# rimelq/VISTAF-RoboSkin-Vision-Integrated-Multimodal-Sensor

Hardware: AMD Instinct MI355X
Metric: frames/sec (224x224 -> force-map) at batch 256 (higher is better)
Workload: dtype f32; 1 GPU; BASELINE configs[2]: batch 256/GPU of 224x224x3 fp16 fringe frames (256 distinct frames) -> 224x224 f32 depth map + force scalars, full FTP path (inpaint, demod, unwrap, detrend, compose, force tail), constants scaled-224; inputs resident in HBM; global_batch=256, input_dtype=fp16, constants=scaled, parallelism=dp1, inflight_batches=3, frames_with_nonzero_status=0

## Files before the change

vistaf-roboskin-vision-integrated-multimodal-sensor_amd/_lib.py:

```python
from __future__ import annotations

import ctypes
import os

_HERE = os.path.dirname(os.path.abspath(__file__))
LIB_PATH = os.path.join(_HERE, "libvistaf_ftp.so")

NSCALARS = 16
NREFINFO = 8
NCONTACT = 16
MAX_CONTACTS = 64
NTRACK = 16
TRACK_NAMES = ["track_id", "age_frames", "parent_row", "events", "overlap_px", "dx", "dy", "dforce_N", "dvolume_cm3", "origin_track_id"]
TRACK_EVENTS = {"born": 1, "split": 2, "merged": 4, "gated": 8}
FATE_ENDED, FATE_NO_ROW = -1, -2 ** 31
NSHAPE = 24
SHAPE_NAMES = ["contact_pixels", "boundary_pixels", "footprint_cx", "footprint_cy", "major_axis_mm", "minor_axis_mm", "orientation_rad",
               "fit_pixels", "fit_status", "apex_x", "apex_y", "apex_depth_mm", "curvature_1_per_mm", "curvature_2_per_mm",
               "curvature_axis_rad", "radius_1_mm", "radius_2_mm", "fit_rms_mm"]
SHAPE_FIT = {"ok": 0, "none": 1, "not_a_cap": 2}
NTAXEL, NTAXELFRAME, TAXEL_NONE = 12, 8, 0xFFFF
TAXEL_NAMES = ["contact_pixels", "contact_area_mm2", "volume_cm3", "mean_depth_mm", "max_depth_mm", "argmax_index", "centroid_x", "centroid_y",
               "force_N", "pressure_kPa"]
TAXEL_FRAME_NAMES = ["active_taxels", "volume_cm3", "force_N", "cop_x", "cop_y", "moment_x_Nmm", "moment_y_Nmm", "peak_taxel"]
NTHERMAL, NTHERMALFRAME = 16, 8
THERMAL_NAMES = ["contact_pixels", "valid_pixels", "coverage", "mean_C", "weighted_mean_C", "min_C", "max_C", "std_C", "peak_temp_C",
                 "surround_pixels", "surround_mean_C", "contrast_C"]
THERMAL_FRAME_NAMES = ["registered_pixels", "skin_mean_C", "contact_pixels", "contact_mean_C", "contrast_C", "hottest_contact", "coldest_contact"]
ALIGN_NINFO = 12

FMT_GRAY_U8, FMT_BGR_U8, FMT_GRAY_F16, FMT_BGR_F16 = 0, 1, 2, 3
FRAME_OK, FRAME_EMPTY_RELIABLE, FRAME_QUEUE_OVERFLOW, FRAME_NO_CARRIER = 0, 1, 2, 3
CURVE_TYPES = {"linear0": 0, "linear": 1, "poly2": 2, "sat_exp": 3, "growth": 4, "hinge_saturating": 5}

EXPORTS = [
    "vistaf_ftp_abi_version", "vistaf_ftp_last_error", "vistaf_ftp_default_config", "vistaf_ftp_create",
    "vistaf_ftp_set_reference", "vistaf_ftp_get_reference_info", "vistaf_ftp_predict_batch", "vistaf_ftp_predict_pairs",
    "vistaf_ftp_get_pair_info", "vistaf_ftp_contacts",
    "vistaf_ftp_get_intermediate", "vistaf_ftp_stage_count", "vistaf_ftp_stage_name",
    "vistaf_ftp_enable_stage_timing", "vistaf_ftp_get_stage_times", "vistaf_ftp_destroy",
    "vistaf_depth_map_to_volume", "vistaf_predict_force_from_volume",
]
TEST_EXPORTS = ["vistaf_ftp_test_set", "vistaf_ftp_test_select", "vistaf_ftp_test_polyfit", "vistaf_ftp_test_gauss",
                "vistaf_ftp_test_chamfer"]
TEMP_EXPORTS = ["vistaf_tempseg_default_config", "vistaf_tempseg_create", "vistaf_tempseg_destroy", "vistaf_tempseg_segment",
                "vistaf_temp_feature_planes", "vistaf_temp_color_support",
                "vistaf_temp_clamp_map", "vistaf_temp_inpaint_map", "vistaf_temp_fuse_maps", "vistaf_temp_oriented_blur"]
TEMPSEG_NINFO = 16
TEMPMODEL_EXPORTS = ["vistaf_tmodel_create", "vistaf_tmodel_destroy", "vistaf_tmodel_predict_maps", "vistaf_tmodel_predict_rows"]
TSENSOR_EXPORTS = ["vistaf_tsensor_default_config", "vistaf_tsensor_create", "vistaf_tsensor_destroy", "vistaf_tsensor_predict",
                   "vistaf_tsensor_stats_create", "vistaf_tsensor_stats_destroy", "vistaf_tsensor_map_statistics"]
TSENSOR_NINFO, TSENSOR_NMASKS, TSENSOR_NSTATS = TEMPSEG_NINFO + 4, 5, 6
TRACK_EXPORTS = ["vistaf_track_create", "vistaf_track_update", "vistaf_track_reset", "vistaf_track_destroy"]
SHAPE_EXPORTS = ["vistaf_shape_create", "vistaf_shape_measure", "vistaf_shape_destroy"]
TAXEL_EXPORTS = ["vistaf_taxel_create", "vistaf_taxel_measure", "vistaf_taxel_layout_info", "vistaf_taxel_destroy"]
THERMAL_EXPORTS = ["vistaf_thermal_create", "vistaf_thermal_register", "vistaf_thermal_measure", "vistaf_thermal_destroy"]
ALIGN_EXPORTS = [
    "vistaf_align_default_config", "vistaf_align_create", "vistaf_align_destroy", "vistaf_align_geometry",
    "vistaf_align_set_reference", "vistaf_align_batch",
]


class Curve(ctypes.Structure):
    _fields_ = [("type", ctypes.c_int32), ("reserved", ctypes.c_int32),
                ("a", ctypes.c_double), ("b", ctypes.c_double), ("c", ctypes.c_double)]

# ... 49 lines not shown
    lib.vistaf_ftp_abi_version.restype = ci
    lib.vistaf_ftp_last_error.restype = ctypes.c_char_p
    lib.vistaf_ftp_default_config.argtypes = [ctypes.POINTER(CConfig)]
    lib.vistaf_ftp_create.argtypes = [ctypes.POINTER(CConfig), ci, ci, ci, ci, ci, ci, ctypes.POINTER(Curve), ci,
                                      ctypes.POINTER(Curve), ctypes.POINTER(vp)]
    lib.vistaf_ftp_set_reference.argtypes = [vp, vp, ci, vp]
    lib.vistaf_ftp_get_reference_info.argtypes = [vp, ctypes.POINTER(cd)]
    lib.vistaf_ftp_predict_batch.argtypes = [vp, vp, ci, ci, vp, vp, vp, vp, vp]
    lib.vistaf_ftp_predict_pairs.argtypes = [vp, vp, vp, ci, ci, vp, vp, vp, vp, vp]
    lib.vistaf_ftp_get_pair_info.argtypes = [vp, ci, ctypes.POINTER(cd), vp]
    lib.vistaf_ftp_contacts.argtypes = [vp, ci, ci, vp, vp, vp, vp]
    lib.vistaf_ftp_get_intermediate.argtypes = [vp, ctypes.c_char_p, vp, ci, ctypes.POINTER(ctypes.c_size_t), vp]
    lib.vistaf_ftp_stage_count.restype = ci
    lib.vistaf_ftp_stage_name.restype = ctypes.c_char_p
    lib.vistaf_ftp_stage_name.argtypes = [ci]
    lib.vistaf_ftp_enable_stage_timing.argtypes = [vp, ci]
    lib.vistaf_ftp_get_stage_times.argtypes = [vp, ctypes.POINTER(ctypes.c_float), ci]
    lib.vistaf_ftp_destroy.argtypes = [vp]
    lib.vistaf_ftp_destroy.restype = None
    lib.vistaf_depth_map_to_volume.argtypes = [vp, vp, ci, ci, ci, cd, cd, vp, vp]
    lib.vistaf_predict_force_from_volume.argtypes = [ctypes.POINTER(Curve), cd, ctypes.POINTER(cd)]
    lib.vistaf_ftp_test_set.argtypes = [vp, ctypes.c_char_p, ci]
    lib.vistaf_ftp_test_select.argtypes = [vp, vp, ctypes.c_size_t, vp, ci, vp, ci, vp, vp, ci, ci, ci, vp]
    lib.vistaf_ftp_test_polyfit.argtypes = [vp, vp, ci, ci, ctypes.c_float, ci, ci, vp, vp, ci, ci, ci, ci, vp]
    lib.vistaf_ftp_test_gauss.argtypes = [vp, vp, cd, ci, ci, ci, vp]
    lib.vistaf_ftp_test_chamfer.argtypes = [vp, ci, ci, vp, vp, ci, ci, ci, ci, vp]
    lib.vistaf_tempseg_default_config.argtypes = [ctypes.POINTER(CTempSegConfig)]
    lib.vistaf_tempseg_create.argtypes = [ctypes.POINTER(CTempSegConfig), ci, ci, ctypes.POINTER(vp)]
    lib.vistaf_tempseg_destroy.argtypes = [vp]
    lib.vistaf_tempseg_destroy.restype = None
    lib.vistaf_tempseg_segment.argtypes = [vp, vp, vp, vp, vp, vp, vp, ctypes.POINTER(cd), vp]
    lib.vistaf_temp_feature_planes.argtypes = [vp, vp, ci, vp, vp, vp, vp, vp]
    lib.vistaf_temp_color_support.argtypes = [vp, vp, vp, vp, vp, vp, cd, ci, vp, vp, vp]
    lib.vistaf_temp_clamp_map.argtypes = [vp, vp, vp, cd, cd, vp, vp]
    lib.vistaf_temp_inpaint_map.argtypes = [vp, vp, vp, ci, vp, vp]
    lib.vistaf_temp_fuse_maps.argtypes = [vp, vp, vp, vp, ctypes.POINTER(CTempFuseConfig), vp, vp, ctypes.POINTER(ctypes.c_int64), vp]
    lib.vistaf_temp_oriented_blur.argtypes = [vp, vp, vp, cd, cd, cd, vp, vp]
    i32p, dp = ctypes.POINTER(ctypes.c_int32), ctypes.POINTER(cd)
    lib.vistaf_tmodel_create.argtypes = [ci, i32p, dp, dp, ci, ci, ci, i32p, dp, cd, ci, dp, dp, cd, cd, ci, ctypes.POINTER(vp)]
    lib.vistaf_tmodel_destroy.argtypes = [vp]
    lib.vistaf_tmodel_destroy.restype = None
    lib.vistaf_tmodel_predict_maps.argtypes = [ci, ctypes.POINTER(vp), ctypes.POINTER(vp), ctypes.POINTER(vp), ctypes.POINTER(vp), ctypes.c_int64,
                                               ctypes.c_int64, vp]
    lib.vistaf_tmodel_predict_rows.argtypes = [vp, vp, ci, ctypes.c_int64, vp, vp]
    lib.vistaf_tsensor_default_config.argtypes = [ctypes.POINTER(CTSensorConfig)]
    lib.vistaf_tsensor_create.argtypes = [ctypes.POINTER(CTSensorConfig), ci, ci, vp, vp, ctypes.POINTER(vp)]
# ... 40 lines not shown
```

vistaf-roboskin-vision-integrated-multimodal-sensor_amd/csrc/api.hip:

```cpp
#include <hip/hip_runtime.h>
#include <algorithm>
#include <cmath>
#include <cstdio>
#include <cstdlib>
#include <cstring>
#include <map>
#include <string>
#include <vector>

#include "host_util.hpp"

using namespace vf;
#include "test_hooks.h"
#ifdef VISTAF_DEBUG
namespace vf { void telea_debug_dump(); void telea_window_debug_dump(int B); void telea_window_mw_debug_dump(int B); void fit_debug_dump(); void unwrap_big_debug_dump(); void unwrap_batch_debug_dump(); }
#endif

static thread_local std::string g_err;
static int fail(int code, const std::string &msg) { g_err = msg; return code; }
namespace vf { int set_error(int code, const std::string &msg) { return fail(code, msg); } }

namespace {

struct GKern { float *d = nullptr; int k = 0; };
// ... 35 lines not shown
    struct Named { void *p; size_t bytes; bool per_frame; };
    std::map<std::string, Named> named;
    DeviceAllocs allocs;
    float *img, *grad, *tmpf, *blurA, *inorm, *iw, *amp, *prod, *quality, *wrapped, *unwrapped, *phase1, *resid0, *detr, *z0, *mplane,
        *num, *den, *hmap, *dist, *z0f, *snum, *unitless, *depth;
    double2 *field, *patch;
    double2 *tmpT;
    uint8_t *bad0, *bad1, *rel0, *rel1, *rel2, *reliable, *contact, *contact_d, *background, *cand, *kept;
    uint8_t *out_rel = nullptr, *hole_cand = nullptr;
    float *hole_med = nullptr, *hole_fill = nullptr;
    int32_t *labels, *area, *rowdist, *parent;
    unsigned int *peak_bits;
    uint16_t *morph_pre;
    void *inpaint_scratch, *inpaint_cl_scratch, *inpaint_win_scratch, *unwrap_scratch;
    void *big_scratch = nullptr;
    int32_t *unwrap_need;
    float *thr_hi, *thr_g, *mu, *amp_thr, *thr3, *thr_used, *bg_med, *core_thr, *core_med, *coef;
    int *cnt_a, *cnt_valid, *rel_count, *contact_count, *bg_count, *bad_count, *flipped;
    unsigned int *gmax;
    int32_t *status;
    int32_t *big_only;
    unsigned long long *cc_best;
    double *scalars;
    float *req_hi, *req_g, *req_med, *req_amp, *req_contact, *req_core;

    ContactScratch contacts_ws{};
    int last_batch = 0;
    bool last_pairs = false;

    bool timing = false;
    hipEvent_t ev[ST_COUNT + 1];
    bool ev_made = false;
    float stage_ms[ST_COUNT];
};

namespace {

template <typename T>
int dalloc(vistaf_ftp_handle *hd, T **p, size_t count, const char *name = nullptr, size_t per_frame = 0)
{
    const int rc = hd->allocs.alloc(p, count);
    if (!rc && name) hd->named[name] = {*p, per_frame, true};
    return rc;
}

int make_gkern(vistaf_ftp_handle *hd, double sigma, GKern *g)
{
// ... 49 lines not shown
void *chain_scratch(const vistaf_ftp_handle *hd) { return hd->tiers.big_chain ? hd->big_scratch : nullptr; }

float q32_of(double pct) { return (float)pct / 100.0f; }

int upload_req(vistaf_ftp_handle *hd, float **d, const std::vector<float> &v)
{
    int rc = dalloc(hd, d, v.size());
    if (rc) return rc;
    if (hipMemcpy(*d, v.data(), v.size() * sizeof(float), hipMemcpyHostToDevice) != hipSuccess) return fail(VISTAF_E_HIP, "memcpy req");
    return 0;
}

void preprocess(vistaf_ftp_handle *hd, const void *frames, int format, int nframes, hipStream_t st, bool timed, const void *frames2 = nullptr)
{
    const vistaf_ftp_config &c = hd->cfg;
    int h = hd->h, w = hd->w, P = hd->P;
    if (timed) hipEventRecord(hd->ev[ST_GRAY_BAD], st);
    launch_to_gray(frames, format, hd->img, nframes, P, st);
    if (frames2) launch_to_gray(frames2, format, hd->img + (size_t)nframes * P, nframes, P, st);
    const int B = frames2 ? 2 * nframes : nframes;
    hipMemsetAsync(hd->bad_count, 0, sizeof(int) * B, st);
    if (c.bad_pixel_enable) {
        launch_sobel_mag(hd->img, hd->grad, B, h, w, st);
        launch_select(hd->img, hd->valid, 0, nullptr, false, hd->req_hi, 1, hd->thr_hi, hd->cnt_valid, B, P, st, chain_scratch(hd));
        launch_select(hd->grad, hd->valid, 0, nullptr, false, hd->req_g, 1, hd->thr_g, nullptr, B, P, st, chain_scratch(hd));
        launch_bad_flags(hd->img, hd->grad, hd->valid, hd->thr_hi, hd->thr_g, hd->bad0, B, P, st);
        uint8_t *src = hd->bad0, *dst = hd->bad1;
        if (c.bad_dilate_ksize > 1)
            for (int it = 0; it < c.bad_dilate_iters; it++) { launch_morph(src, dst, B, h, w, hd->se_bad, true, nullptr, nullptr, st); std::swap(src, dst); }
        if (src != hd->bad1) hipMemcpyAsync(hd->bad1, src, (size_t)B * P, hipMemcpyDeviceToDevice, st);
        launch_count_u8(hd->bad1, hd->bad_count, B, P, st);
        {
            int range = std::min(100, std::max(1, cv_round((double)c.bad_inpaint_radius)));
            const uint8_t *seq_mask = hd->bad1;
            const int32_t *only = nullptr;
            int mode = hd->tiers.inpaint;
            if (mode == 2 && (size_t)h * w > (size_t)8 * 14464) mode = 0;
            if (mode == 0 && inpaint_clusters_supported(range)) {
                uint8_t *bad_big = nullptr;
                ClusterPlanes left;
                launch_inpaint_clusters(hd->img, hd->bad1, range, hd->inpaint_cl_scratch, &bad_big, &left, B, h, w, st);
                if (timed) hipEventRecord(hd->ev[ST_INPAINT], st);
                launch_inpaint_big_clusters(hd->img, bad_big, range, hd->inpaint_scratch, hd->status, left, B, h, w, st, hd->tiers.big_queue_lds != 0,
                                            hd->tiers.big_gq_cap);
                if (hd->tiers.big_fallback) {
                    launch_inpaint_big_handback(hd->status, hd->big_only, B, st);
                    launch_inpaint_telea(hd->img, bad_big, range, hd->inpaint_scratch, hd->status, hd->big_only, B, h, w, st);
                }
            } else {
                if (timed && mode == 1) hipEventRecord(hd->ev[ST_INPAINT], st);
                if (mode != 1) only = launch_inpaint_window(hd->img, seq_mask, range, hd->inpaint_win_scratch, B, h, w, st, timed ? hd->ev[ST_INPAINT] : nullptr,
                                                               hd->tiers.telea_two_tier != 0, hd->tiers.telea_mw != 0);
                launch_inpaint_telea(hd->img, seq_mask, range, hd->inpaint_scratch, hd->status, only, B, h, w, st);
            }
        }
    } else if (timed) hipEventRecord(hd->ev[ST_INPAINT], st);
    if (timed) hipEventRecord(hd->ev[ST_PREPROC], st);
    blur(hd, hd->img, hd->blurA, hd->g_illum, B, st);
    if (fuses(hd, hd->g_pre)) launch_illum_pre_apod(hd->img, hd->blurA, hd->apo, hd->iw, hd->g_pre.d, hd->g_pre.k, B, h, w, st);
    else {
        launch_illum_norm(hd->img, hd->blurA, hd->inorm, B, P, st);
        const float *in = hd->inorm;
        if (hd->g_pre.k) { blur(hd, hd->inorm, hd->blurA, hd->g_pre, B, st); in = hd->blurA; }
        launch_mul_static(in, hd->apo, hd->iw, B, P, st);
    }
    launch_select(hd->iw, hd->valid, 0, nullptr, false, hd->req_med, 1, hd->mu, nullptr, B, P, st, chain_scratch(hd));
}

std::vector<float> hann_patch(int ph, int pw)
{
    auto hann = [](int M, int i) -> float { return M == 1 ? 1.0f : (float)(0.5 + 0.5 * std::cos(3.14159265358979323846 * (double)(1 - M + 2 * i) / (double)(M - 1))); };
    std::vector<float> win((size_t)ph * pw);
    for (int a = 0; a < ph; a++)
        for (int c = 0; c < pw; c++) win[(size_t)a * pw + c] = hann(ph, a) * hann(pw, c);
    return win;
}

PostParams post_params(const vistaf_ftp_handle *hd, const CarrierGeom *pair_geom)
{
    PostParams pp;
    pp.mm_per_px = hd->mm_per_px; pp.depth_eps_mm = hd->cfg.depth_eps_mm; pp.period_px = hd->period; pp.force_curve = hd->fcurve;
    pp.pair_geom = pair_geom; pp.grating_pitch_mm = hd->cfg.grating_pitch_mm;
    return pp;
}

void ensure_events(vistaf_ftp_handle *hd)
{
    if (hd->ev_made) return;
    for (int i = 0; i <= ST_COUNT; i++) hipEventCreate(&hd->ev[i]);
// ... 142 lines not shown
    TRY(dalloc(hd, &hd->thr3, mb * 3)); TRY(dalloc(hd, &hd->thr_used, mb)); TRY(dalloc(hd, &hd->bg_med, mb));
    TRY(dalloc(hd, &hd->core_thr, mb)); TRY(dalloc(hd, &hd->core_med, mb)); TRY(dalloc(hd, &hd->coef, mb * 6));
    TRY(dalloc(hd, &hd->cnt_a, mb)); TRY(dalloc(hd, &hd->cnt_valid, mb)); TRY(dalloc(hd, &hd->rel_count, mb));
    TRY(dalloc(hd, &hd->contact_count, mb)); TRY(dalloc(hd, &hd->bg_count, mb)); TRY(dalloc(hd, &hd->bad_count, mb));
    TRY(dalloc(hd, &hd->flipped, mb)); TRY(dalloc(hd, &hd->gmax, mb)); TRY(dalloc(hd, &hd->status, mb)); TRY(dalloc(hd, &hd->cc_best, mb));
    TRY(dalloc(hd, &hd->big_only, mb));
    TRY(dalloc(hd, &hd->scalars, mb * VISTAF_NSCALARS));
    TRY(dalloc(hd, &hd->hole_med, mb)); TRY(dalloc(hd, &hd->hole_fill, mb));
    {
        ContactScratch &cs = hd->contacts_ws;
        cs.cap = contact_root_capacity(h, w);
        TRY(dalloc(hd, &cs.arg, n)); TRY(dalloc(hd, &cs.list, mb * cs.cap)); TRY(dalloc(hd, &cs.nroots, mb)); TRY(dalloc(hd, &cs.nsel, mb));
        TRY(dalloc(hd, &cs.selkey, mb * VISTAF_MAX_CONTACTS)); TRY(dalloc(hd, &cs.part, contact_part_words(max_batch, P)));
    }
    hd->named["mu"] = {hd->mu, sizeof(float), true}; hd->named["thr_hi"] = {hd->thr_hi, sizeof(float), true}; hd->named["thr_g"] = {hd->thr_g, sizeof(float), true};
    hd->named["coef"] = {hd->coef, 6 * sizeof(float), true}; hd->named["thr3"] = {hd->thr3, 3 * sizeof(float), true};
    hd->named["core_thr"] = {hd->core_thr, sizeof(float), true}; hd->named["core_med"] = {hd->core_med, sizeof(float), true};
    TRY(upload_req(hd, &hd->req_hi, {q32_of(cfg->bad_intensity_percentile)}));
    TRY(upload_req(hd, &hd->req_g, {q32_of(cfg->bad_gradient_percentile)}));
    TRY(upload_req(hd, &hd->req_med, {-1.0f}));
    TRY(upload_req(hd, &hd->req_amp, {q32_of(cfg->amp_valid_percentile)}));
    TRY(upload_req(hd, &hd->req_contact, {q32_of(cfg->contact_percentile), q32_of(95.0), q32_of(98.0)}));
    TRY(upload_req(hd, &hd->req_core, {q32_of(cfg->contact_core_percentile)}));
    TRY(dalloc(hd, &hd->roi_den, (size_t)P));
    if (hd->g_unrel.k) {
        float *tmp_roi = nullptr;
        TRY(upload(hd, &tmp_roi, roif));
        launch_gauss_rows(tmp_roi, hd->tmpf, hd->g_unrel.d, hd->g_unrel.k, 1, h, w, 0);
        launch_gauss_cols(hd->tmpf, hd->roi_den, hd->g_unrel.d, hd->g_unrel.k, 1, h, w, 0);
        std::vector<float> hden(P);
        if (hipMemcpy(hden.data(), hd->roi_den, P * sizeof(float), hipMemcpyDeviceToHost) != hipSuccess) { vistaf_ftp_destroy(hd); return fail(VISTAF_E_HIP, "roi_den readback"); }
        for (int i = 0; i < P; i++) hden[i] = hden[i] + 1e-6f;
        if (hipMemcpy(hd->roi_den, hden.data(), P * sizeof(float), hipMemcpyHostToDevice) != hipSuccess) { vistaf_ftp_destroy(hd); return fail(VISTAF_E_HIP, "roi_den upload"); }
    }
    hd->Hf = h + 2 * std::max(0, cfg->fft_pad_px);
    hd->Wf = w + 2 * std::max(0, cfg->fft_pad_px);
    if (hipDeviceSynchronize() != hipSuccess) { vistaf_ftp_destroy(hd); return fail(VISTAF_E_HIP, "create sync"); }
#undef TRY
    *out = hd;
    return 0;
}

static int reference_search(vistaf_ftp_handle *hd, int nb, CarrierGeom *geom_dev, hipStream_t st)
{
    const vistaf_ftp_config &c = hd->cfg;
    const int h = hd->h, w = hd->w, Hf = hd->Hf, Wf = hd->Wf, pad = std::max(0, c.fft_pad_px);
// ... 55 lines not shown
    return 0;
}

int vistaf_ftp_get_reference_info(const vistaf_ftp_handle *hd, double *o)
{
    if (!hd || !o) return fail(VISTAF_E_INVALID, "null argument");
    if (!hd->have_ref) return fail(VISTAF_E_STATE, "set_reference has not been called");
    o[0] = hd->peak_x; o[1] = hd->peak_y; o[2] = hd->kx; o[3] = hd->ky; o[4] = hd->Hf; o[5] = hd->Wf; o[6] = hd->period; o[7] = hd->mm_per_px;
    return 0;
}

static int post_demod(vistaf_ftp_handle *hd, int B, float *d_height_mm, uint8_t *d_reliable, double *d_scalars, int32_t *d_status,
                      const CarrierGeom *pair_geom, hipStream_t st, const int *bad_count = nullptr)
{
    if (!bad_count) bad_count = hd->bad_count;
    const vistaf_ftp_config &c = hd->cfg;
    int h = hd->h, w = hd->w, P = hd->P;
    bool timed = hd->timing;

    if (timed) hipEventRecord(hd->ev[ST_RELIABLE], st);
    if (hd->g_qual.k) blur(hd, hd->prod, hd->quality, hd->g_qual, B, st);
    else HIPCHK(hipMemcpyAsync(hd->quality, hd->prod, (size_t)B * P * sizeof(float), hipMemcpyDeviceToDevice, st));
    const float *qual = hd->quality;
    launch_select(qual, hd->roi, 0, nullptr, false, hd->req_amp, 1, hd->amp_thr, nullptr, B, P, st, chain_scratch(hd));
    launch_threshold_mask(qual, hd->roi, hd->amp_thr, hd->rel0, B, P, st);
    {
        uint8_t *src = hd->rel0, *dst = hd->rel1;
        if (c.valid_close_iters >= 1 && 2 * c.valid_close_iters <= 4) {
            int ops[4];
            for (int it = 0; it < c.valid_close_iters; it++) { ops[it] = 1; ops[c.valid_close_iters + it] = 0; }
            launch_morph_seq(hd->rel0, hd->rel1, hd->rel2, B, h, w, hd->se_close, ops, 2 * c.valid_close_iters, hd->roi, nullptr, st, hd->morph_pre);
            src = hd->rel1;
        } else {
            for (int it = 0; it < 2 * c.valid_close_iters; it++) {
                const bool dil = it < c.valid_close_iters;
                launch_morph(src, dst, B, h, w, hd->se_close, dil, it == 2 * c.valid_close_iters - 1 ? hd->roi : nullptr, nullptr, st, hd->morph_pre);
                src = dst;
                dst = dst == hd->rel1 ? hd->rel2 : hd->rel1;
            }
        }
        launch_cc_label(src, hd->labels, B, h, w, st);
        launch_cc_largest(hd->labels, hd->area, hd->cc_best, hd->roi, hd->rel2, B, P, st);
    }
    if (c.reliable_edge_margin_px > 0) {
        RowSpanSE ball;
        if (chamfer_ball((float)c.reliable_edge_margin_px, &ball))
            launch_morph(hd->rel2, hd->reliable, B, h, w, ball, false, nullptr, nullptr, st, hd->morph_pre);
        else {
            launch_chamfer(hd->rel2, false, hd->rowdist, hd->dist, B, h, w, c.reliable_edge_margin_px + 1, st, hd->tiers.chamfer_twopass != 0);
            launch_erode_by_dist(hd->dist, hd->rel2, (float)c.reliable_edge_margin_px, hd->reliable, B, P, st);
        }
    } else HIPCHK(hipMemcpyAsync(hd->reliable, hd->rel2, (size_t)B * P, hipMemcpyDeviceToDevice, st));
    launch_count_u8(hd->reliable, hd->rel_count, B, P, st);
    launch_mark_empty(hd->rel_count, hd->status, B, st);

    if (timed) hipEventRecord(hd->ev[ST_UNWRAP_RANK], st);
    launch_unwrap(hd->wrapped, qual, hd->reliable, hd->unwrapped, hd->parent, hd->unwrap_scratch, hd->status, B, h, w, st,
                  timed ? hd->ev[ST_UNWRAP_TREE] : nullptr, timed ? hd->ev[ST_UNWRAP] : nullptr, hd->tiers.big_flood_handback != 0, hd->tiers.unwrap_fast ? hd->unwrap_need : nullptr);

    if (timed) hipEventRecord(hd->ev[ST_DETREND], st);
    if (c.plane_order_for_removal > 0)
        launch_robust_polyfit(hd->unwrapped, hd->reliable, c.plane_order_for_removal, c.irls_iters, (float)c.irls_c, 200, 500, hd->coef, hd->phase1, B, h, w, st, chain_scratch(hd));
    else
        HIPCHK(hipMemcpyAsync(hd->phase1, hd->unwrapped, (size_t)B * P * sizeof(float), hipMemcpyDeviceToDevice, st));
    launch_robust_polyfit(hd->phase1, hd->reliable, c.poly_order, c.irls_iters, (float)c.irls_c, 200, 0, hd->coef, hd->resid0, B, h, w, st, chain_scratch(hd));
    launch_select(hd->resid0, hd->reliable, (size_t)P, nullptr, true, hd->req_contact, 3, hd->thr3, nullptr, B, P, st, chain_scratch(hd));
    launch_contact_mask(hd->resid0, hd->reliable, hd->thr3, hd->rel_count, hd->contact_count, c.min_contact_frac, c.max_contact_frac,
                        hd->contact, hd->thr_used, B, P, st);
    {
        int iters = c.dilate_iters;
        if (iters <= 0) HIPCHK(hipMemcpyAsync(hd->contact_d, hd->contact, (size_t)B * P, hipMemcpyDeviceToDevice, st));
        else if (iters <= 4) {
            int ops[4] = {1, 1, 1, 1};
            launch_morph_seq(hd->contact, hd->contact_d, hd->cand, B, h, w, hd->se_contact, ops, iters, nullptr, hd->reliable, st, hd->morph_pre);
        } else {
            uint8_t *src = hd->contact, *dst = hd->contact_d;
            uint8_t *bufs[2] = {hd->contact_d, hd->cand};
            for (int it = 0; it < iters; it++) {
                dst = bufs[it & 1];
                launch_morph(src, dst, B, h, w, hd->se_contact, true, nullptr, it == iters - 1 ? hd->reliable : nullptr, st, hd->morph_pre);
                src = dst;
            }
            if (src != hd->contact_d) HIPCHK(hipMemcpyAsync(hd->contact_d, src, (size_t)B * P, hipMemcpyDeviceToDevice, st));
        }
    }
    launch_background(hd->reliable, hd->contact_d, hd->rel_count, hd->bg_count, hd->background, B, P, st);
    launch_robust_polyfit(hd->phase1, hd->background, c.poly_order, c.irls_iters, (float)c.irls_c, 200, 0, hd->coef, hd->detr, B, h, w, st, chain_scratch(hd));
    launch_select(hd->detr, hd->background, (size_t)P, nullptr, false, hd->req_med, 1, hd->bg_med, nullptr, B, P, st, chain_scratch(hd));

    if (timed) hipEventRecord(hd->ev[ST_SMOOTH_FLIP], st);
    const bool smooth_rel = hd->g_rel.k > 0;
    if (fuses(hd, hd->g_rel)) launch_smooth_reliable(hd->detr, hd->bg_med, hd->reliable, hd->hmap, hd->g_rel.d, hd->g_rel.k, B, h, w, st);
    else if (smooth_rel) {
        launch_sub_scalar_mask(hd->detr, hd->bg_med, hd->reliable, hd->z0, hd->mplane, B, P, st);
        blur(hd, hd->z0, hd->num, hd->g_rel, B, st);
        blur(hd, hd->mplane, hd->den, hd->g_rel, B, st);
        launch_div_planes(hd->num, hd->den, hd->hmap, B, P, st);
    } else launch_zeroed_keep_nan(hd->detr, hd->bg_med, hd->reliable, hd->hmap, B, P, st);
    launch_select(hd->hmap, hd->reliable, (size_t)P, nullptr, false, hd->req_core, 1, hd->core_thr, nullptr, B, P, st, chain_scratch(hd));
    launch_select(hd->hmap, hd->reliable, (size_t)P, hd->core_thr, false, hd->req_med, 1, hd->core_med, nullptr, B, P, st, chain_scratch(hd));
    launch_core_flip(hd->hmap, hd->core_med, hd->flipped, B, P, st);

    const uint8_t *orel = hd->reliable;
    if (!smooth_rel) {
        const int ksz = std::max(3, c.hole_neighborhood_px | 1);
        launch_chamfer(hd->reliable, false, hd->rowdist, hd->dist, B, h, w, c.hole_min_dist_px + 1, st, hd->tiers.chamfer_twopass != 0);
        launch_hole_candidates(hd->hmap, hd->reliable, hd->dist, ksz, (float)c.hole_known_fraction, (float)c.hole_min_dist_px, hd->hole_cand, B, h, w, st);
        launch_select(hd->hmap, hd->reliable, (size_t)P, nullptr, false, hd->req_med, 1, hd->hole_med, nullptr, B, P, st, chain_scratch(hd));
        launch_hole_tmp(hd->hmap, hd->reliable, hd->hole_cand, hd->hole_med, hd->z0, B, P, st);
        launch_select(hd->z0, hd->reliable, (size_t)P, nullptr, false, hd->req_med, 1, hd->hole_fill, nullptr, B, P, st, chain_scratch(hd));
        launch_hole_zin(hd->z0, hd->hole_fill, B, P, st);
        {
            const int range = std::min(100, std::max(1, cv_round((double)c.inpaint_radius)));
            const int32_t *only = nullptr;
            if (hd->tiers.inpaint != 1) only = launch_inpaint_window(hd->z0, hd->hole_cand, range, hd->inpaint_win_scratch, B, h, w, st, nullptr, hd->tiers.telea_two_tier != 0, hd->tiers.telea_mw != 0);
            launch_inpaint_telea(hd->z0, hd->hole_cand, range, hd->inpaint_scratch, hd->status, only, B, h, w, st);
        }
        launch_hole_merge(hd->hmap, hd->reliable, hd->hole_cand, hd->z0, hd->out_rel, B, P, st);
        orel = hd->out_rel;
    }

    if (timed) hipEventRecord(hd->ev[ST_COMPOSE], st);
    bool use_band = c.frontier_zero_band_px > 0;
    float band = (float)c.frontier_zero_band_px;
    if (use_band) launch_chamfer_pair(orel, hd->rowdist, hd->dist, hd->area, hd->depth, B, h, w, c.frontier_zero_band_px + 2, st, hd->tiers.chamfer_twopass != 0);
    else HIPCHK(hipMemsetAsync(hd->dist, 0x7f, (size_t)B * P * sizeof(float), st));
    const bool fuse_compose = fuses(hd, hd->g_unrel);
    if (fuse_compose)
        launch_compose_finalize_mm(hd->hmap, orel, hd->roi, hd->dist, use_band ? band : 1.0f, hd->roi_den, use_band ? hd->depth : hd->dist, band,
                                   use_band ? 1 : 0, hd->hcurve, hd->use_neg, hd->unitless, hd->depth, hd->cand, hd->gmax, hd->g_unrel.d, hd->g_unrel.k,
                                   B, h, w, st);
    else {
        launch_frontier_compose(hd->hmap, orel, hd->roi, hd->dist, use_band ? band : 1.0f, hd->z0f, B, P, st);
// ... 158 lines not shown
    return 0;
}
int vistaf_ftp_get_stage_times(vistaf_ftp_handle *hd, float *ms_out, int n)
{
    if (!hd || !ms_out) return fail(VISTAF_E_INVALID, "null argument");
    for (int i = 0; i < n && i < ST_COUNT; i++) ms_out[i] = hd->stage_ms[i];
    return 0;
}

int vistaf_ftp_test_set(vistaf_ftp_handle *hd, const char *name, int value)
{
    if (!hd || !name) return fail(VISTAF_E_INVALID, "null argument");
    const std::string n(name);
    if (n == "inpaint_tier" && value >= 0 && value <= 2) hd->tiers.inpaint = value;
    else if (n == "big_flood_handback") hd->tiers.big_flood_handback = value != 0;
    else if (n == "chamfer_twopass") hd->tiers.chamfer_twopass = value != 0;
    else if (n == "telea_two_tier") hd->tiers.telea_two_tier = value != 0;
    else if (n == "telea_mw") hd->tiers.telea_mw = value != 0;
    else if (n == "big_queue_lds") hd->tiers.big_queue_lds = value != 0;
    else if (n == "big_gq_cap" && (value == 0 || (value >= 64 && (value & (value - 1)) == 0))) hd->tiers.big_gq_cap = value;
    else if (n == "big_fallback") hd->tiers.big_fallback = value != 0;
    else if (n == "unwrap_fast") hd->tiers.unwrap_fast = value != 0;
    else if (n == "big_chain") hd->tiers.big_chain = value != 0;
    else if (n == "fused_chains") hd->tiers.fused_chains = value != 0;
    else if (n == "fused_backend") hd->tiers.fused_backend = value != 0;
    else if (n == "keep_planes") hd->keep_planes = value != 0;
    else return fail(VISTAF_E_INVALID, "unknown test hook or value: " + n);
    return 0;
}

namespace {
int hook_scratch(int variant, int B, int h, int w, bool chain_ok, void **scratch)
{
    *scratch = nullptr;
    if (variant < 0 || variant > 2) return fail(VISTAF_E_INVALID, "variant must be 0, 1 or 2");
    if (variant == 2 && !chain_ok) return fail(VISTAF_E_INVALID, "variant 2: the k_big.hip chain does not take this batch");
    if (variant == 1 || (variant == 0 && (size_t)h * w < 262144)) return 0;
    HIPCHK(hipMalloc(scratch, big_scratch_bytes(B, h, w) + 256));
    return 0;
}
int hook_finish(void *a, void *b, hipStream_t st)
{
    const hipError_t e1 = hipGetLastError(), e2 = hipStreamSynchronize(st);
    if (a) (void)hipFree(a);
    if (b) (void)hipFree(b);
    if (e1 != hipSuccess) return fail(VISTAF_E_HIP, std::string("launch: ") + hipGetErrorString(e1));
    if (e2 != hipSuccess) return fail(VISTAF_E_HIP, std::string("sync: ") + hipGetErrorString(e2));
    return 0;
}
}

int vistaf_ftp_test_select(const float *vals, const uint8_t *mask, size_t mask_stride, const float *le_thr, int use_abs, const float *reqs, int nreq,
                           float *out, int *counts, int B, int P, int variant, void *stream)
{
    if (!vals || !mask || !reqs || !out || B < 1 || P < 1 || nreq < 1 || (mask_stride != 0 && mask_stride != (size_t)P))
        return fail(VISTAF_E_INVALID, "bad argument");
    void *scratch = nullptr;
    int rc = hook_scratch(variant, B, 1, P, nreq <= 4 && big_frames(B, P), &scratch);
    if (rc) return rc;
    launch_select(vals, mask, mask_stride, le_thr, use_abs != 0, reqs, nreq, out, counts, B, P, (hipStream_t)stream, scratch);
    return hook_finish(scratch, nullptr, (hipStream_t)stream);
}

int vistaf_ftp_test_polyfit(const float *z, const uint8_t *mask, int order, int iters, float c, int min_count, int min_mask_count, float *coef,
                            float *resid, int B, int h, int w, int variant, void *stream)
{
    if (!z || !mask || !coef || !resid || B < 1 || h < 1 || w < 1 || (size_t)h * w > 0x7fffffffull || order < 1 || order > 2 || iters < 1)
        return fail(VISTAF_E_INVALID, "bad argument");
    void *scratch = nullptr;
    int rc = hook_scratch(variant, B, h, w, big_frames(B, h * w), &scratch);
    if (rc) return rc;
    const int inst = polyfit_variant(B, h, w, scratch != nullptr);
    launch_robust_polyfit(z, mask, order, iters, c, min_count, min_mask_count, coef, resid, B, h, w, (hipStream_t)stream, scratch);
    rc = hook_finish(scratch, nullptr, (hipStream_t)stream);
    return rc ? rc : inst;
}

int vistaf_ftp_test_gauss(const float *src, float *dst, double sigma, int B, int h, int w, void *stream)
{
    if (!src || !dst || src == dst || B < 1 || h < 1 || w < 1 || !(sigma > 0)) return fail(VISTAF_E_INVALID, "bad argument");
    if (gauss_ksize(sigma) > 511) return fail(VISTAF_E_INVALID, "gaussian sigma too large (ksize > 511)");
    const std::vector<float> f = gauss_taps(sigma);
    float *taps = nullptr, *tmp = nullptr;
    HIPCHK(hipMalloc((void **)&taps, f.size() * sizeof(float)));
// ... 44 lines not shown
```

vistaf-roboskin-vision-integrated-multimodal-sensor_amd/csrc/k_select.hip:

```cpp
#include "kernels.hpp"
#include "select.hpp"

namespace vf {

struct PlaneGetter {
    const float *v; const uint8_t *m; float le; bool use_le, use_abs;
    __device__ bool operator()(int i, uint32_t &key) const
    {
        const uint8_t mk = m[i];
        float x = v[i];
        bool ok = mk != 0 && finitef(x);
        if (use_abs) x = fabsf(x);
        if (use_le && !(x <= le)) ok = false;
        key = f2key(x);
        return ok;
    }
};

__global__ __launch_bounds__(SEL_T) void k_select(const float *__restrict__ vals, const uint8_t *__restrict__ mask, size_t mask_stride,
                                                  const float *__restrict__ le_thr, int use_abs, const float *__restrict__ reqs,
                                                  int nreq, float *__restrict__ out, int *__restrict__ counts, int P)
{
    __shared__ SelShared sh;
    size_t b = blockIdx.x;
    PlaneGetter g{vals + b * (size_t)P, mask + b * mask_stride, le_thr ? le_thr[b] : 0.f, le_thr != nullptr, use_abs != 0};
    uint32_t n, kmin, kmax;
    block_minmax(g, P, sh, n, kmin, kmax);
    if (threadIdx.x == 0 && counts) counts[b] = (int)n;
    for (int j = 0; j < nreq; j++) {
        float q = reqs[j];
        float r = (q < 0.f) ? block_median(g, P, sh, n, kmin, kmax) : block_percentile(g, P, q, sh, n, kmin, kmax);
        if (threadIdx.x == 0) out[b * (size_t)nreq + j] = r;
        __syncthreads();
    }
}

void launch_select(const float *vals, const uint8_t *mask, size_t mask_stride, const float *le_thr, bool use_abs,
                   const float *reqs_dev, int nreq, float *out, int *counts, int B, int P, hipStream_t st, void *big_scratch)
{
    if (big_scratch && nreq <= 4 && big_frames(B, P)) {
        launch_select_big(vals, mask, mask_stride, le_thr, use_abs, reqs_dev, nreq, out, counts, B, P, big_scratch, st);
        return;
    }
    hipLaunchKernelGGL(k_select, dim3(B), dim3(SEL_T), 0, st, vals, mask, mask_stride, le_thr, use_abs ? 1 : 0, reqs_dev, nreq,
                       out, counts, P);
}

}
```

vistaf-roboskin-vision-integrated-multimodal-sensor_amd/csrc/kernels.hpp:

```cpp
#pragma once
#include <hip/hip_runtime.h>
#include <stdint.h>
#include "common.hpp"

namespace vf {

struct Tiers {
    int inpaint = 2;
    int big_flood_handback = 0;
    int chamfer_twopass = 0;
    int telea_two_tier = 1;
    int unwrap_fast = 1;
    int big_chain = 1;
    int big_queue_lds = 1;
    int big_gq_cap = 0;
    int big_fallback = 1;
    int telea_mw = 1;
    int fused_backend = 1;
    int fused_chains = 1;
};

struct RowSpanSE {
    int k;
    int8_t lo[33];
    int8_t hi[33];
};

void launch_to_gray(const void *frames, int format, float *gray, int B, int P, hipStream_t st);
void launch_sobel_mag(const float *img, float *grad, int B, int h, int w, hipStream_t st);
void launch_bad_flags(const float *img, const float *grad, const uint8_t *valid, const float *thr_hi, const float *thr_g,
                      uint8_t *bad, int B, int P, hipStream_t st);
void launch_morph(const uint8_t *src, uint8_t *dst, int B, int h, int w, const RowSpanSE &se, bool dilate,
                  const uint8_t *and_static, const uint8_t *and_frame, hipStream_t st, uint16_t *prefix_scratch = nullptr);
void launch_morph_seq(const uint8_t *src, uint8_t *dst, uint8_t *tmp, int B, int h, int w, const RowSpanSE &se, const int *dilates, int n,
                      const uint8_t *and_static, const uint8_t *and_frame, hipStream_t st, uint16_t *prefix_scratch = nullptr);
void launch_gauss_rows(const float *src, float *dst, const float *kern, int ksize, int B, int h, int w, hipStream_t st);
void launch_gauss_blur(const float *src, float *tmp, float *dst, const float *kern, int ksize, int B, int h, int w, hipStream_t st);
void launch_gauss_cols(const float *src, float *dst, const float *kern, int ksize, int B, int h, int w, hipStream_t st);
void launch_illum_norm(const float *img, const float *blur, float *out, int B, int P, hipStream_t st);
void launch_mul_static(const float *a, const float *stat, float *out, int B, int P, hipStream_t st);
void launch_count_u8(const uint8_t *m, int *counts, int B, int P, hipStream_t st);

constexpr int GF_MAXK = 15;

void launch_illum_pre_apod(const float *img, const float *blur_illum, const float *apo, float *iw, const float *kern, int ksize, int B, int h,
                           int w, hipStream_t st);
void launch_smooth_reliable(const float *detr, const float *bg_med, const uint8_t *reliable, float *hmap, const float *kern, int ksize, int B,
                            int h, int w, hipStream_t st);
void launch_compose_finalize_mm(const float *hmap, const uint8_t *reliable, const uint8_t *roi, const float *dist_in, float taper_band,
                                const float *roi_den, const float *dist_out, float band, int use_band, Curve curve, int use_neg, float *unitless,
                                float *depth, uint8_t *cand, unsigned int *gmax_bits, const float *kern, int ksize, int B, int h, int w,
                                hipStream_t st);

void launch_select(const float *vals, const uint8_t *mask, size_t mask_stride, const float *le_thr, bool use_abs,
                   const float *reqs_dev, int nreq, float *out, int *counts, int B, int P, hipStream_t st, void *big_scratch = nullptr);

struct CarrierGeom {
    double peak_x, peak_y;
    double kx, ky;
    double dpx, dpy;
    double period;
    int x0, y0, ph, pw;
    int px_i, py_i;
    int px_raw, py_raw;
    int ok;
    int keep_carrier;
};
void launch_dft_forward(const float *iw, const float *mu, const double2 *Ex, const double2 *Ey, size_t tab_stride_x, size_t tab_stride_y,
                        const float *win, double2 *tmpT, double2 *patch, int patch_stride, int B, int h, int w, int ph, int pw, hipStream_t st,
                        int win_stride = 0);
void launch_dft_inverse(const double2 *patch, int patch_stride, const double2 *Gx, const double2 *Gy, size_t tab_stride_x, size_t tab_stride_y,
                        double2 *tmpQ, double2 *field, float *amp, const double2 *cref, const float *amp_ref, size_t ref_stride, float *prod,
                        float *wrapped, int B, int h, int w, int ph, int pw, hipStream_t st, const CarrierGeom *geom = nullptr);
void launch_dft_full_mag(const float *iw, const float *mu, const double2 *Ex_full, const double2 *Ey_full, double2 *tmp,
                         double *mag, int B, int h, int w, int Hf, int Wf, hipStream_t st);
void launch_top_peaks(const double *mag, int B, int Hf, int Wf, int dc, int npeaks, double *out_xyv , hipStream_t st);
void launch_carrier_choose(const double *peaks, int npk, const double *mag, int Hf, int Wf, int bw, double max_dy_frac, CarrierGeom *geom, int B,
                           hipStream_t st);
// ... 141 lines not shown
```

Baseline: 70030 frames/s.

## Add register-resident percentile select kernel and chain core threshold with median

Adds a select kernel variant that loads each frame's masked plane once into per-thread registers (16/32/49/64 keys per thread, sized to the plane) and runs the radix-style selection from registers instead of re-streaming the plane from global memory on each pass. Every launch_select call in the FTP path uses it by default via a new select_resident tier flag. The core threshold and the median below that threshold, which used to be two separate launches, now run as one chained launch that reuses the resident keys. The cost is heavy register pressure: a 224x224 plane needs 49 keys per thread, which may spill or cut occupancy, and with only one block per frame there is limited parallelism.

```diff
diff --git a/vistaf-roboskin-vision-integrated-multimodal-sensor_amd/_lib.py b/vistaf-roboskin-vision-integrated-multimodal-sensor_amd/_lib.py
--- a/vistaf-roboskin-vision-integrated-multimodal-sensor_amd/_lib.py
+++ b/vistaf-roboskin-vision-integrated-multimodal-sensor_amd/_lib.py
@@ -41,7 +41,7 @@
     "vistaf_ftp_enable_stage_timing", "vistaf_ftp_get_stage_times", "vistaf_ftp_destroy",
     "vistaf_depth_map_to_volume", "vistaf_predict_force_from_volume",
 ]
-TEST_EXPORTS = ["vistaf_ftp_test_set", "vistaf_ftp_test_select", "vistaf_ftp_test_polyfit", "vistaf_ftp_test_gauss",
+TEST_EXPORTS = ["vistaf_ftp_test_set", "vistaf_ftp_test_select", "vistaf_ftp_test_select_instance", "vistaf_ftp_test_select_chained", "vistaf_ftp_test_polyfit", "vistaf_ftp_test_gauss",
                 "vistaf_ftp_test_chamfer"]
 TEMP_EXPORTS = ["vistaf_tempseg_default_config", "vistaf_tempseg_create", "vistaf_tempseg_destroy", "vistaf_tempseg_segment",
                 "vistaf_temp_feature_planes", "vistaf_temp_color_support",
@@ -137,6 +137,8 @@
     lib.vistaf_predict_force_from_volume.argtypes = [ctypes.POINTER(Curve), cd, ctypes.POINTER(cd)]
     lib.vistaf_ftp_test_set.argtypes = [vp, ctypes.c_char_p, ci]
     lib.vistaf_ftp_test_select.argtypes = [vp, vp, ctypes.c_size_t, vp, ci, vp, ci, vp, vp, ci, ci, ci, vp]
+    lib.vistaf_ftp_test_select_instance.argtypes = [ci, ci, ci, ci]
+    lib.vistaf_ftp_test_select_chained.argtypes = [vp, vp, ctypes.c_size_t, ci, vp, ci, vp, vp, ci, ci, vp]
     lib.vistaf_ftp_test_polyfit.argtypes = [vp, vp, ci, ci, ctypes.c_float, ci, ci, vp, vp, ci, ci, ci, ci, vp]
     lib.vistaf_ftp_test_gauss.argtypes = [vp, vp, cd, ci, ci, ci, vp]
     lib.vistaf_ftp_test_chamfer.argtypes = [vp, ci, ci, vp, vp, ci, ci, ci, ci, vp]
diff --git a/vistaf-roboskin-vision-integrated-multimodal-sensor_amd/csrc/api.hip b/vistaf-roboskin-vision-integrated-multimodal-sensor_amd/csrc/api.hip
--- a/vistaf-roboskin-vision-integrated-multimodal-sensor_amd/csrc/api.hip
+++ b/vistaf-roboskin-vision-integrated-multimodal-sensor_amd/csrc/api.hip
@@ -81,7 +81,7 @@
     int32_t *big_only;
     unsigned long long *cc_best;
     double *scalars;
-    float *req_hi, *req_g, *req_med, *req_amp, *req_contact, *req_core;
+    float *req_hi, *req_g, *req_med, *req_amp, *req_contact, *req_core, *req_core_med;
 
     ContactScratch contacts_ws{};
     int last_batch = 0;
@@ -177,8 +177,8 @@
     hipMemsetAsync(hd->bad_count, 0, sizeof(int) * B, st);
     if (c.bad_pixel_enable) {
         launch_sobel_mag(hd->img, hd->grad, B, h, w, st);
-        launch_select(hd->img, hd->valid, 0, nullptr, false, hd->req_hi, 1, hd->thr_hi, hd->cnt_valid, B, P, st, chain_scratch(hd));
-        launch_select(hd->grad, hd->valid, 0, nullptr, false, hd->req_g, 1, hd->thr_g, nullptr, B, P, st, chain_scratch(hd));
+        launch_select(hd->img, hd->valid, 0, nullptr, false, hd->req_hi, 1, hd->thr_hi, hd->cnt_valid, B, P, st, chain_scratch(hd), hd->tiers.select_resident != 0);
+        launch_select(hd->grad, hd->valid, 0, nullptr, false, hd->req_g, 1, hd->thr_g, nullptr, B, P, st, chain_scratch(hd), hd->tiers.select_resident != 0);
         launch_bad_flags(hd->img, hd->grad, hd->valid, hd->thr_hi, hd->thr_g, hd->bad0, B, P, st);
         uint8_t *src = hd->bad0, *dst = hd->bad1;
         if (c.bad_dilate_ksize > 1)
@@ -219,7 +219,7 @@
         if (hd->g_pre.k) { blur(hd, hd->inorm, hd->blurA, hd->g_pre, B, st); in = hd->blurA; }
         launch_mul_static(in, hd->apo, hd->iw, B, P, st);
     }
-    launch_select(hd->iw, hd->valid, 0, nullptr, false, hd->req_med, 1, hd->mu, nullptr, B, P, st, chain_scratch(hd));
+    launch_select(hd->iw, hd->valid, 0, nullptr, false, hd->req_med, 1, hd->mu, nullptr, B, P, st, chain_scratch(hd), hd->tiers.select_resident != 0);
 }
 
 std::vector<float> hann_patch(int ph, int pw)
@@ -408,6 +408,7 @@
     TRY(upload_req(hd, &hd->req_amp, {q32_of(cfg->amp_valid_percentile)}));
     TRY(upload_req(hd, &hd->req_contact, {q32_of(cfg->contact_percentile), q32_of(95.0), q32_of(98.0)}));
     TRY(upload_req(hd, &hd->req_core, {q32_of(cfg->contact_core_percentile)}));
+    TRY(upload_req(hd, &hd->req_core_med, {q32_of(cfg->contact_core_percentile), -1.0f}));
     TRY(dalloc(hd, &hd->roi_den, (size_t)P));
     if (hd->g_unrel.k) {
         float *tmp_roi = nullptr;
@@ -509,7 +510,7 @@
     if (hd->g_qual.k) blur(hd, hd->prod, hd->quality, hd->g_qual, B, st);
     else HIPCHK(hipMemcpyAsync(hd->quality, hd->prod, (size_t)B * P * sizeof(float), hipMemcpyDeviceToDevice, st));
     const float *qual = hd->quality;
-    launch_select(qual, hd->roi, 0, nullptr, false, hd->req_amp, 1, hd->amp_thr, nullptr, B, P, st, chain_scratch(hd));
+    launch_select(qual, hd->roi, 0, nullptr, false, hd->req_amp, 1, hd->amp_thr, nullptr, B, P, st, chain_scratch(hd), hd->tiers.select_resident != 0);
     launch_threshold_mask(qual, hd->roi, hd->amp_thr, hd->rel0, B, P, st);
     {
         uint8_t *src = hd->rel0, *dst = hd->rel1;
@@ -551,7 +552,7 @@
     else
         HIPCHK(hipMemcpyAsync(hd->phase1, hd->unwrapped, (size_t)B * P * sizeof(float), hipMemcpyDeviceToDevice, st));
     launch_robust_polyfit(hd->phase1, hd->reliable, c.poly_order, c.irls_iters, (float)c.irls_c, 200, 0, hd->coef, hd->resid0, B, h, w, st, chain_scratch(hd));
-    launch_select(hd->resid0, hd->reliable, (size_t)P, nullptr, true, hd->req_contact, 3, hd->thr3, nullptr, B, P, st, chain_scratch(hd));
+    launch_select(hd->resid0, hd->reliable, (size_t)P, nullptr, true, hd->req_contact, 3, hd->thr3, nullptr, B, P, st, chain_scratch(hd), hd->tiers.select_resident != 0);
     launch_contact_mask(hd->resid0, hd->reliable, hd->thr3, hd->rel_count, hd->contact_count, c.min_contact_frac, c.max_contact_frac,
                         hd->contact, hd->thr_used, B, P, st);
     {
@@ -573,7 +574,7 @@
     }
     launch_background(hd->reliable, hd->contact_d, hd->rel_count, hd->bg_count, hd->background, B, P, st);
     launch_robust_polyfit(hd->phase1, hd->background, c.poly_order, c.irls_iters, (float)c.irls_c, 200, 0, hd->coef, hd->detr, B, h, w, st, chain_scratch(hd));
-    launch_select(hd->detr, hd->background, (size_t)P, nullptr, false, hd->req_med, 1, hd->bg_med, nullptr, B, P, st, chain_scratch(hd));
+    launch_select(hd->detr, hd->background, (size_t)P, nullptr, false, hd->req_med, 1, hd->bg_med, nullptr, B, P, st, chain_scratch(hd), hd->tiers.select_resident != 0);
 
     if (timed) hipEventRecord(hd->ev[ST_SMOOTH_FLIP], st);
     const bool smooth_rel = hd->g_rel.k > 0;
@@ -584,8 +585,12 @@
         blur(hd, hd->mplane, hd->den, hd->g_rel, B, st);
         launch_div_planes(hd->num, hd->den, hd->hmap, B, P, st);
     } else launch_zeroed_keep_nan(hd->detr, hd->bg_med, hd->reliable, hd->hmap, B, P, st);
-    launch_select(hd->hmap, hd->reliable, (size_t)P, nullptr, false, hd->req_core, 1, hd->core_thr, nullptr, B, P, st, chain_scratch(hd));
-    launch_select(hd->hmap, hd->reliable, (size_t)P, hd->core_thr, false, hd->req_med, 1, hd->core_med, nullptr, B, P, st, chain_scratch(hd));
+    float *const core_outs[2] = {hd->core_thr, hd->core_med};
+    if (select_variant(B, P, 2, chain_scratch(hd) != nullptr, hd->tiers.select_resident != 0) < SELV_RES16 ||
+        launch_select_chained(hd->hmap, hd->reliable, (size_t)P, false, hd->req_core_med, 2, core_outs, nullptr, B, P, st) < 0) {
+        launch_select(hd->hmap, hd->reliable, (size_t)P, nullptr, false, hd->req_core, 1, hd->core_thr, nullptr, B, P, st, chain_scratch(hd), hd->tiers.select_resident != 0);
+        launch_select(hd->hmap, hd->reliable, (size_t)P, hd->core_thr, false, hd->req_med, 1, hd->core_med, nullptr, B, P, st, chain_scratch(hd), hd->tiers.select_resident != 0);
+    }
     launch_core_flip(hd->hmap, hd->core_med, hd->flipped, B, P, st);
 
     const uint8_t *orel = hd->reliable;
@@ -593,9 +598,9 @@
         const int ksz = std::max(3, c.hole_neighborhood_px | 1);
         launch_chamfer(hd->reliable, false, hd->rowdist, hd->dist, B, h, w, c.hole_min_dist_px + 1, st, hd->tiers.chamfer_twopass != 0);
         launch_hole_candidates(hd->hmap, hd->reliable, hd->dist, ksz, (float)c.hole_known_fraction, (float)c.hole_min_dist_px, hd->hole_cand, B, h, w, st);
-        launch_select(hd->hmap, hd->reliable, (size_t)P, nullptr, false, hd->req_med, 1, hd->hole_med, nullptr, B, P, st, chain_scratch(hd));
+        launch_select(hd->hmap, hd->reliable, (size_t)P, nullptr, false, hd->req_med, 1, hd->hole_med, nullptr, B, P, st, chain_scratch(hd), hd->tiers.select_resident != 0);
         launch_hole_tmp(hd->hmap, hd->reliable, hd->hole_cand, hd->hole_med, hd->z0, B, P, st);
-        launch_select(hd->z0, hd->reliable, (size_t)P, nullptr, false, hd->req_med, 1, hd->hole_fill, nullptr, B, P, st, chain_scratch(hd));
+        launch_select(hd->z0, hd->reliable, (size_t)P, nullptr, false, hd->req_med, 1, hd->hole_fill, nullptr, B, P, st, chain_scratch(hd), hd->tiers.select_resident != 0);
         launch_hole_zin(hd->z0, hd->hole_fill, B, P, st);
         {
             const int range = std::min(100, std::max(1, cv_round((double)c.inpaint_radius)));
@@ -800,6 +805,7 @@
     else if (n == "big_fallback") hd->tiers.big_fallback = value != 0;
     else if (n == "unwrap_fast") hd->tiers.unwrap_fast = value != 0;
     else if (n == "big_chain") hd->tiers.big_chain = value != 0;
+    else if (n == "select_resident") hd->tiers.select_resident = value != 0;
     else if (n == "fused_chains") hd->tiers.fused_chains = value != 0;
     else if (n == "fused_backend") hd->tiers.fused_backend = value != 0;
     else if (n == "keep_planes") hd->keep_planes = value != 0;
@@ -833,11 +839,32 @@
 {
     if (!vals || !mask || !reqs || !out || B < 1 || P < 1 || nreq < 1 || (mask_stride != 0 && mask_stride != (size_t)P))
         return fail(VISTAF_E_INVALID, "bad argument");
+    if (variant < 0 || variant > 3) return fail(VISTAF_E_INVALID, "variant must be 0, 1, 2 or 3");
     void *scratch = nullptr;
-    int rc = hook_scratch(variant, B, 1, P, nreq <= 4 && big_frames(B, P), &scratch);
+    int rc = hook_scratch(variant == 3 ? 1 : variant, B, 1, P, nreq <= 4 && big_frames(B, P), &scratch);
     if (rc) return rc;
-    launch_select(vals, mask, mask_stride, le_thr, use_abs != 0, reqs, nreq, out, counts, B, P, (hipStream_t)stream, scratch);
+    launch_select(vals, mask, mask_stride, le_thr, use_abs != 0, reqs, nreq, out, counts, B, P, (hipStream_t)stream, scratch, variant != 3);
     return hook_finish(scratch, nullptr, (hipStream_t)stream);
+}
+
+int vistaf_ftp_test_select_instance(int B, int P, int nreq, int variant)
+{
+    if (B < 1 || P < 1 || nreq < 1 || variant < 0 || variant > 3) return fail(VISTAF_E_INVALID, "bad argument");
+    const bool chain_ok = nreq <= 4 && big_frames(B, P);
+    if (variant == 2 && !chain_ok) return fail(VISTAF_E_INVALID, "variant 2: the k_big.hip chain does not take this batch");
+    return select_variant(B, P, nreq, variant == 2 || (variant == 0 && P >= 262144), variant != 3);
+}
+
+int vistaf_ftp_test_select_chained(const float *vals, const uint8_t *mask, size_t mask_stride, int use_abs, const float *reqs, int nreq, float *out,
+                                   int *counts, int B, int P, void *stream)
+{
+    if (!vals || !mask || !reqs || !out || B < 1 || P < 1 || nreq < 1 || nreq > 4 || (mask_stride != 0 && mask_stride != (size_t)P))
+        return fail(VISTAF_E_INVALID, "bad argument");
+    float *outs[4] = {out, out + B, out + 2 * (size_t)B, out + 3 * (size_t)B};
+    const int inst = launch_select_chained(vals, mask, mask_stride, use_abs != 0, reqs, nreq, outs, counts, B, P, (hipStream_t)stream);
+    if (inst < 0) return fail(VISTAF_E_INVALID, "no resident instance takes this plane size");
+    const int rc = hook_finish(nullptr, nullptr, (hipStream_t)stream);
+    return rc ? rc : inst;
 }
 
 int vistaf_ftp_test_polyfit(const float *z, const uint8_t *mask, int order, int iters, float c, int min_count, int min_mask_count, float *coef,
diff --git a/vistaf-roboskin-vision-integrated-multimodal-sensor_amd/csrc/k_select.hip b/vistaf-roboskin-vision-integrated-multimodal-sensor_amd/csrc/k_select.hip
--- a/vistaf-roboskin-vision-integrated-multimodal-sensor_amd/csrc/k_select.hip
+++ b/vistaf-roboskin-vision-integrated-multimodal-sensor_amd/csrc/k_select.hip
@@ -35,15 +35,132 @@
     }
 }
 
+constexpr uint32_t SEL_NOKEY = 0xFFFFFFFFu;
+constexpr int SEL_MAX_CHAIN = 4;
+struct SelOut { float *p[SEL_MAX_CHAIN]; };
+
+template <int NS>
+__device__ inline void resident_minmax(const uint32_t (&key)[NS], uint32_t cut, SelShared &sh, uint32_t &n, uint32_t &kmin, uint32_t &kmax)
+{
+    uint32_t c = 0, mn = SEL_NOKEY, mx = 0;
+#pragma unroll
+    for (int s = 0; s < NS; s++)
+        if (key[s] <= cut) { c++; mn = key[s] < mn ? key[s] : mn; mx = key[s] > mx ? key[s] : mx; }
+    __syncthreads();
+    n = block_sum<uint32_t>(c, sh.wsum);
+    kmin = (uint32_t)block_min_u64(mn, sh.red64);
+    kmax = (uint32_t)block_max_u64(mx, sh.red64);
+    __syncthreads();
+}
+
+template <int NS>
+__global__ __launch_bounds__(SEL_T) void k_select_resident(const float *__restrict__ vals, const uint8_t *__restrict__ mask, size_t mask_stride,
+                                                           const float *__restrict__ le_thr, int use_abs, const float *__restrict__ reqs,
+                                                           int nreq, int chained, SelOut out, int *__restrict__ counts, int P)
+{
+    __shared__ SelShared sh;
+    const size_t b = blockIdx.x;
+    const PlaneGetter g{vals + b * (size_t)P, mask + b * mask_stride, le_thr ? le_thr[b] : 0.f, le_thr != nullptr, use_abs != 0};
+    uint32_t key[NS];
+#pragma unroll
+    for (int s0 = 0; s0 < NS; s0 += SEL_U) {
+        bool ok[SEL_U];
+#pragma unroll
+        for (int u = 0; u < SEL_U; u++)
+            if (s0 + u < NS) {
+                const int i = (int)threadIdx.x + (s0 + u) * SEL_T;
+                ok[u] = g(i < P ? i : P - 1, key[s0 + u]) && i < P;
+            }
+#pragma unroll
+        for (int u = 0; u < SEL_U; u++)
+            if (s0 + u < NS && !ok[u]) key[s0 + u] = SEL_NOKEY;
+    }
+    uint32_t cut = SEL_NOKEY - 1u;
+    const auto each = [&](auto body) {
+#pragma unroll
+        for (int s = 0; s < NS; s++) {
+            uint32_t k = key[s];
+            asm volatile("" : "+v"(k));
+            if (k <= cut) body(k);
+        }
+    };
+    uint32_t n, kmin, kmax;
+    resident_minmax<NS>(key, cut, sh, n, kmin, kmax);
+    if (threadIdx.x == 0 && counts) counts[b] = (int)n;
+    float r = 0.f;
+    for (int j = 0; j < nreq; j++) {
+        if (chained && j > 0 && n > 0) {
+            if (r != r) n = 0;
+            else {
+                const uint32_t c2 = f2key(r == 0.f ? 0.f : r);
+                cut = c2 < cut ? c2 : cut;
+                resident_minmax<NS>(key, cut, sh, n, kmin, kmax);
+            }
+        }
+        const float q = reqs[j];
+        const bool median = q < 0.f;
+        uint32_t k = 0; float gm = 0.f; bool top;
+        if (median) k = (n & 1u) ? (n - 1) / 2 : n / 2 - 1;
+        else if (n > 0) np_percentile_index(n, q, k, gm, top);
+        if (n == 0) r = nanf32();
+        else if (median && n == 1) r = key2f(kmin);
+        else if (!median && k + 1 >= n) r = key2f(kmax);
+        else {
+            uint32_t ka, kb;
+            block_select2_each<SEL_T>(each, n, k, sh, kmin, kmax, ka, kb);
+            if (median) r = (n & 1u) ? key2f(ka) : __fdiv_rn(__fadd_rn(key2f(ka), key2f(kb)), 2.0f);
+            else r = np_lerp(key2f(ka), key2f(kb), gm);
+        }
+        if (threadIdx.x == 0) {
+            if (chained) (j == 0 ? out.p[0] : j == 1 ? out.p[1] : j == 2 ? out.p[2] : out.p[3])[b] = r;
+            else out.p[0][b * (size_t)nreq + j] = r;
+        }
+        __syncthreads();
+    }
+}
+
+int select_variant(int B, int P, int nreq, bool big, bool resident)
+{
+    if (big && nreq <= 4 && big_frames(B, P)) return SELV_BIG;
+    if (!resident || P > 64 * SEL_T) return SELV_STREAM;
+    return P <= 16 * SEL_T ? SELV_RES16 : P <= 32 * SEL_T ? SELV_RES32 : P <= 49 * SEL_T ? SELV_RES49 : SELV_RES64;
+}
+
+static void launch_resident(int variant, const float *vals, const uint8_t *mask, size_t mask_stride, const float *le_thr, bool use_abs,
+                            const float *reqs_dev, int nreq, bool chained, const SelOut &out, int *counts, int B, int P, hipStream_t st)
+{
+#define VF_SEL_RES(NS) hipLaunchKernelGGL(k_select_resident<NS>, dim3(B), dim3(SEL_T), 0, st, vals, mask, mask_stride, le_thr, use_abs ? 1 : 0, \
+                                          reqs_dev, nreq, chained ? 1 : 0, out, counts, P)
+    switch (variant) {
+    case SELV_RES16: VF_SEL_RES(16); break;
+    case SELV_RES32: VF_SEL_RES(32); break;
+    case SELV_RES49: VF_SEL_RES(49); break;
+    default: VF_SEL_RES(64); break;
+    }
+#undef VF_SEL_RES
+}
+
 void launch_select(const float *vals, const uint8_t *mask, size_t mask_stride, const float *le_thr, bool use_abs,
-                   const float *reqs_dev, int nreq, float *out, int *counts, int B, int P, hipStream_t st, void *big_scratch)
+                   const float *reqs_dev, int nreq, float *out, int *counts, int B, int P, hipStream_t st, void *big_scratch, bool resident)
 {
-    if (big_scratch && nreq <= 4 && big_frames(B, P)) {
+    const int variant = select_variant(B, P, nreq, big_scratch != nullptr, resident);
+    if (variant == SELV_BIG)
         launch_select_big(vals, mask, mask_stride, le_thr, use_abs, reqs_dev, nreq, out, counts, B, P, big_scratch, st);
-        return;
-    }
-    hipLaunchKernelGGL(k_select, dim3(B), dim3(SEL_T), 0, st, vals, mask, mask_stride, le_thr, use_abs ? 1 : 0, reqs_dev, nreq,
-                       out, counts, P);
+    else if (variant == SELV_STREAM)
+        hipLaunchKernelGGL(k_select, dim3(B), dim3(SEL_T), 0, st, vals, mask, mask_stride, le_thr, use_abs ? 1 : 0, reqs_dev, nreq,
+                           out, counts, P);
+    else launch_resident(variant, vals, mask, mask_stride, le_thr, use_abs, reqs_dev, nreq, false, SelOut{{out}}, counts, B, P, st);
+}
+
+int launch_select_chained(const float *vals, const uint8_t *mask, size_t mask_stride, bool use_abs, const float *reqs_dev, int nreq,
+                          float *const *outs, int *counts, int B, int P, hipStream_t st)
+{
+    const int variant = select_variant(B, P, nreq, false, true);
+    if (variant < SELV_RES16 || nreq < 1 || nreq > SEL_MAX_CHAIN) return -1;
+    SelOut o{};
+    for (int j = 0; j < nreq; j++) o.p[j] = outs[j];
+    launch_resident(variant, vals, mask, mask_stride, nullptr, use_abs, reqs_dev, nreq, true, o, counts, B, P, st);
+    return variant;
 }
 
 }
diff --git a/vistaf-roboskin-vision-integrated-multimodal-sensor_amd/csrc/kernels.hpp b/vistaf-roboskin-vision-integrated-multimodal-sensor_amd/csrc/kernels.hpp
--- a/vistaf-roboskin-vision-integrated-multimodal-sensor_amd/csrc/kernels.hpp
+++ b/vistaf-roboskin-vision-integrated-multimodal-sensor_amd/csrc/kernels.hpp
@@ -17,6 +17,7 @@
     int big_fallback = 1;
     int telea_mw = 1;
     int fused_backend = 1;
+    int select_resident = 1;
     int fused_chains = 1;
 };
 
@@ -53,7 +54,12 @@
                                 hipStream_t st);
 
 void launch_select(const float *vals, const uint8_t *mask, size_t mask_stride, const float *le_thr, bool use_abs,
-                   const float *reqs_dev, int nreq, float *out, int *counts, int B, int P, hipStream_t st, void *big_scratch = nullptr);
+                   const float *reqs_dev, int nreq, float *out, int *counts, int B, int P, hipStream_t st, void *big_scratch = nullptr,
+                   bool resident = true);
+enum SelectVariant { SELV_BIG = 0, SELV_STREAM, SELV_RES16, SELV_RES32, SELV_RES49, SELV_RES64, SELV_COUNT };
+int select_variant(int B, int P, int nreq, bool big, bool resident);
+int launch_select_chained(const float *vals, const uint8_t *mask, size_t mask_stride, bool use_abs, const float *reqs_dev, int nreq,
+                          float *const *outs, int *counts, int B, int P, hipStream_t st);
 
 struct CarrierGeom {
     double peak_x, peak_y;
```

New measurement: 71960 frames/s (median of 6 runs). +2.7%, better.
